# DefTruth/CUDA-Learn-Notes

Hardware: NVIDIA H100
Metric: hgemm_tflops (higher is better)
Workload: dtype f16 (fp32 accumulate)

## Files before the change

### cuda-learn-notes_b200/csrc/hgemm_wgmma.cu

```cuda
#include "abi_common.cuh"
#include "ptx.cuh"

namespace b200k {

namespace gemm {
constexpr int BM = 128, BN = 256, STAGES = 4, THREADS = 384, GROUP_M = 16;
constexpr int STG_BYTES = 16384;
}

template <int DT_, bool A_MN_, bool B_MN_>
struct GemmCfg {
  static constexpr int DT = DT_;
  static constexpr bool A_MN = A_MN_, B_MN = B_MN_;
  static constexpr int ES = DT == 2 ? 4 : 2;
  static constexpr int BK = 128 / ES;
  static constexpr int KSTEP = DT == 2 ? 8 : 16;
  static constexpr int A_BYTES = gemm::BM * BK * ES;
  static constexpr int B_BYTES = gemm::BN * BK * ES;
  static constexpr int STAGE_BYTES = A_BYTES + B_BYTES;
  static constexpr int SMEM_BYTES = gemm::STAGES * STAGE_BYTES + 2 * gemm::STG_BYTES + 1024 + 2 * gemm::STAGES * 8;
  static_assert(!(DT == 2 && (A_MN || B_MN)), "tf32 wgmma reads K-major operands only");
  static_assert(SMEM_BYTES <= 232448, "more shared memory than an H100 block may use");
};

template <class Cfg>
__device__ __forceinline__ void gemm_mma_kblock(float* d, uint32_t sA, uint32_t sB, int cw) {
  constexpr int STEPS = Cfg::BK / Cfg::KSTEP;
#pragma unroll
  for (int k = 0; k < STEPS; ++k) {
    const uint64_t da = Cfg::A_MN ? wgmma_desc(sA + cw * 64 * Cfg::BK * Cfg::ES + k * 2048, 64 * Cfg::BK * Cfg::ES, 1024)
                                  : wgmma_desc(sA + cw * 64 * 128 + k * 32, 16, 1024);
    const uint64_t db = Cfg::B_MN ? wgmma_desc(sB + k * 2048, 64 * Cfg::BK * Cfg::ES, 1024) : wgmma_desc(sB + k * 32, 16, 1024);
    wgmma_ss<Cfg::DT, 256, Cfg::A_MN, Cfg::B_MN>(d, da, db, 1);
  }
}

template <class Cfg>
__device__ __forceinline__ void gemm_store_tile(const float* d, const CUtensorMap* tmC, uint32_t stg, int cw, int row0,
                                                int col0) {
  constexpr int SLICES = Cfg::DT == 2 ? 4 : 2, JS = 32 / SLICES, JB = JS / 2;
  const int t = threadIdx.x & 127, lane = t & 31, warp = t / 32;
  const bool leader = t == 0;
#pragma unroll
  for (int sl = 0; sl < SLICES; ++sl) {
    if (leader) tma_store_wait_read<0>();
    named_bar_sync(1 + cw, 128);
    if constexpr (Cfg::DT == 2) {
      const int q = lane & 3;
#pragma unroll
      for (int jj = 0; jj < JS; ++jj) {
        const int j = sl * JS + jj;
#pragma unroll
        for (int h = 0; h < 2; ++h) {
          const int r = warp * 16 + 8 * h + lane / 4;
          const int chunk = 2 * (jj % JB) + q / 2;
          const uint32_t a = stg + (jj / JB) * 8192 + r * 128 + ((chunk ^ (r & 7)) << 4) + (q & 1) * 8;
          asm volatile("st.shared.v2.f32 [%0], {%1, %2};" ::"r"(a), "f"(d[4 * j + 2 * h]), "f"(d[4 * j + 2 * h + 1])
                       : "memory");
        }
      }
    } else {
      const int m = lane / 8, r = warp * 16 + 8 * (m & 1) + (lane & 7);
#pragma unroll
      for (int jj = 0; jj < JS; jj += 2) {
        const int j = sl * JS + jj, chunk = jj % JB + (m >> 1);
        const uint32_t a = stg + (jj / JB) * 8192 + r * 128 + ((chunk ^ (r & 7)) << 4);
        uint32_t p[4];
#pragma unroll
        for (int i = 0; i < 4; ++i)
          p[i] = Cfg::DT == 1 ? pack_bf162(d[4 * j + 2 * i], d[4 * j + 2 * i + 1])
                              : pack_half2(d[4 * j + 2 * i], d[4 * j + 2 * i + 1]);
        stmatrix_x4(a, p[0], p[1], p[2], p[3]);
      }
    }
    fence_proxy_async_smem();
    named_bar_sync(1 + cw, 128);
    if (leader) {
      const int c = col0 + sl * (gemm::BN / SLICES);
      tma_store_2d(tmC, stg, c, row0);
      tma_store_2d(tmC, stg + 8192, c + 128 / Cfg::ES, row0);
      tma_store_commit();
    }
  }
}

template <class Cfg>
__global__ void __launch_bounds__(gemm::THREADS, 1)
    hgemm_wgmma_kernel(const __grid_constant__ CUtensorMap tmA, const __grid_constant__ CUtensorMap tmB,
                       const __grid_constant__ CUtensorMap tmC, int K, int tiles_m, int tiles_n) {
  using namespace gemm;
  extern __shared__ uint8_t smem_raw[];
  const uint32_t base = (smem_u32(smem_raw) + 1023) & ~1023u;
  const uint32_t stg0 = base + STAGES * Cfg::STAGE_BYTES;
  const uint32_t full0 = stg0 + 2 * STG_BYTES, empty0 = full0 + STAGES * 8;
  const int wg = threadIdx.x / 128;

  const int tile = blockIdx.x, width = GROUP_M * tiles_n, g = tile / width, first_m = g * GROUP_M;
  const int gsz = min(tiles_m - first_m, GROUP_M);
  const int tm = first_m + (tile % width) % gsz, tn = (tile % width) / gsz;
  const int nkb = (K + Cfg::BK - 1) / Cfg::BK;

  if (threadIdx.x == 0) {
    for (int s = 0; s < STAGES; ++s) {
      mbar_init(full0 + 8 * s, 1);
      mbar_init(empty0 + 8 * s, 2);
    }
    fence_mbar_init();
  }
  __syncthreads();

  if (wg == 0) {
    if (threadIdx.x == 0) {
      tma_prefetch_desc(&tmA);
      tma_prefetch_desc(&tmB);
      for (int kb = 0; kb < nkb; ++kb) {
        const int s = kb % STAGES;
        if (kb >= STAGES) mbar_wait_nocall(empty0 + 8 * s, ((kb / STAGES) - 1) & 1);
        const uint32_t bar = full0 + 8 * s, sA = base + s * Cfg::STAGE_BYTES, sB = sA + Cfg::A_BYTES;
        mbar_arrive_expect_tx(bar, Cfg::STAGE_BYTES);
        if constexpr (Cfg::A_MN) {
#pragma unroll
          for (int c = 0; c < BM / 64; ++c)
            tma_load_2d(sA + c * 64 * Cfg::BK * Cfg::ES, &tmA, bar, tm * BM + c * 64, kb * Cfg::BK, kPolicyEvictNormal);
        } else {
          tma_load_2d(sA, &tmA, bar, kb * Cfg::BK, tm * BM, kPolicyEvictNormal);
        }
        if constexpr (Cfg::B_MN) {
#pragma unroll
          for (int c = 0; c < BN / 64; ++c)
            tma_load_2d(sB + c * 64 * Cfg::BK * Cfg::ES, &tmB, bar, tn * BN + c * 64, kb * Cfg::BK, kPolicyEvictNormal);
        } else {
          tma_load_2d(sB, &tmB, bar, kb * Cfg::BK, tn * BN, kPolicyEvictNormal);
        }
      }
    }
    return;
  }

  const int cw = wg - 1, t = threadIdx.x & 127;
  const bool leader = t == 0;
  if (leader) tma_prefetch_desc(&tmC);
  float d[128];
#pragma unroll
  for (int i = 0; i < 128; ++i) d[i] = 0.f;
  for (int kb = 0; kb < nkb; ++kb) {
    const int s = kb % STAGES;
    mbar_wait_nocall(full0 + 8 * s, (kb / STAGES) & 1);
    const uint32_t sA = base + s * Cfg::STAGE_BYTES, sB = sA + Cfg::A_BYTES;
    fence_regs<128>(d);
    wgmma_fence();
    gemm_mma_kblock<Cfg>(d, sA, sB, cw);
    wgmma_commit();
    wgmma_wait<1>();
    fence_regs<128>(d);
    if (kb > 0 && leader) mbar_arrive(empty0 + 8 * ((kb - 1) % STAGES));
  }
  wgmma_wait<0>();
  fence_regs<128>(d);
  gemm_store_tile<Cfg>(d, &tmC, stg0 + cw * STG_BYTES, cw, tm * BM + cw * 64, tn * BN);
  if (leader) tma_store_wait_all<0>();
}

template <class Cfg>
static int launch_gemm(const void* A, const void* B, void* C, int64_t M, int64_t N, int64_t K, cudaStream_t s,
                       const DeviceInfo& di) {
  using namespace gemm;
  auto tmap = [](CUtensorMap* m, const void* p, int64_t rows, int64_t cols, uint32_t box_rows, uint32_t box_cols) {
    const uint64_t dims[2] = {uint64_t(cols), uint64_t(rows)}, strides[1] = {uint64_t(cols) * Cfg::ES};
    const uint32_t box[2] = {box_cols, box_rows};
    return make_tmap(m, p, Cfg::ES, 2, dims, strides, box);
  };
  CUtensorMap tmA, tmB, tmC;
  int rc = Cfg::A_MN ? tmap(&tmA, A, K, M, Cfg::BK, 64) : tmap(&tmA, A, M, K, BM, Cfg::BK);
  if (rc) return rc;
  rc = Cfg::B_MN ? tmap(&tmB, B, K, N, Cfg::BK, 64) : tmap(&tmB, B, N, K, BN, Cfg::BK);
  if (rc) return rc;
  if ((rc = tmap(&tmC, C, M, N, 64, 128 / Cfg::ES))) return rc;
  const int64_t tiles_m = (M + BM - 1) / BM, tiles_n = (N + BN - 1) / BN, tiles = tiles_m * tiles_n;
  if (tiles > INT32_MAX) return set_error(B200K_ESHAPE, "GEMM too large: %lld tiles", (long long)tiles);
  auto kern = hgemm_wgmma_kernel<Cfg>;
  if ((rc = ensure_dynamic_smem(reinterpret_cast<const void*>(kern), di.device, Cfg::SMEM_BYTES))) return rc;
  kern<<<unsigned(tiles), THREADS, Cfg::SMEM_BYTES, s>>>(tmA, tmB, tmC, int(K), int(tiles_m), int(tiles_n));
  B200K_CHECK_CUDA(cudaGetLastError());
  return B200K_OK;
}

template <int DT>
static int gemm_dispatch(const char* who, const void* A, const void* B, void* C, int64_t M, int64_t N, int64_t K,
                         int b_is_nk, int variant, void* stream, int a_is_km = 0) {
  constexpr int PACK = (DT == 2) ? 4 : 8;
  if (!A || !B || !C) return set_error(B200K_EARG, "%s: null pointer", who);
  if (reinterpret_cast<uintptr_t>(C) & 15) return set_error(B200K_EALIGN, "%s: C (%p) must be 16-byte aligned", who, C);
  if (M < 1 || N < 1 || K < 1 || M > INT32_MAX || N > INT32_MAX || K > INT32_MAX)
    return set_error(B200K_ESHAPE, "%s: M,N,K must be in [1, 2^31) (got %lld,%lld,%lld)", who, (long long)M, (long long)N,
                     (long long)K);
  if ((K % PACK) || (N % PACK))
    return set_error(B200K_ESHAPE, "%s: K and N must be multiples of %d (16-byte rows), got K=%lld N=%lld", who, PACK,
                     (long long)K, (long long)N);
  if (a_is_km && DT == 2) return set_error(B200K_EDTYPE, "%s: A stored as [K,M] is built for f16 / bf16 only", who);
  if (a_is_km && (M % PACK))
    return set_error(B200K_ESHAPE, "%s: M must be a multiple of %d when A is stored as [K,M]", who, PACK);
  const int v = variant & 0xff;
  if (v < B200K_HGEMM_AUTO || v > B200K_HGEMM_2CTA_512x256)
    return set_error(B200K_EARG, "%s: variant %d unknown", who, v);
  DeviceInfo di;
  int rc = get_device_info(&di);
  if (rc) return rc;
  cudaStream_t s = static_cast<cudaStream_t>(stream);
  const bool nn = (b_is_nk == 0);
  if constexpr (DT == 2) {
    if (!nn) return launch_gemm<GemmCfg<2, false, false>>(A, B, C, M, N, K, s, di);
    void* bt = nullptr;
    B200K_CHECK_CUDA(cudaMallocAsync(&bt, size_t(K) * size_t(N) * 4, s));
    rc = b200k_mat_transpose_f32(B, bt, K, N, stream);
    if (!rc) rc = launch_gemm<GemmCfg<2, false, false>>(A, bt, C, M, N, K, s, di);
    cudaError_t e = cudaFreeAsync(bt, s);
    if (!rc && e != cudaSuccess) rc = set_error(B200K_ECUDA, "cudaFreeAsync failed: %s", cudaGetErrorString(e));
    return rc;
  } else {
    if (a_is_km)
      return nn ? launch_gemm<GemmCfg<DT, true, true>>(A, B, C, M, N, K, s, di)
                : launch_gemm<GemmCfg<DT, true, false>>(A, B, C, M, N, K, s, di);
    return nn ? launch_gemm<GemmCfg<DT, false, true>>(A, B, C, M, N, K, s, di)
              : launch_gemm<GemmCfg<DT, false, false>>(A, B, C, M, N, K, s, di);
  }
}

}

extern "C" int b200k_hgemm_f16(const void* A, const void* B, void* C, int64_t M, int64_t N, int64_t K, int b_is_nk,
                               int variant, void* stream) {
  return b200k::gemm_dispatch<0>("b200k_hgemm_f16", A, B, C, M, N, K, b_is_nk, variant, stream);
}

extern "C" int b200k_gemm_ex(const void* A, const void* B, void* C, int64_t M, int64_t N, int64_t K, int a_is_km, int b_is_nk,
                             int dtype, int variant, void* stream) {
  switch (dtype) {
    case B200K_F16: return b200k::gemm_dispatch<0>("b200k_gemm_ex(f16)", A, B, C, M, N, K, b_is_nk, variant, stream, a_is_km);
    case B200K_BF16: return b200k::gemm_dispatch<1>("b200k_gemm_ex(bf16)", A, B, C, M, N, K, b_is_nk, variant, stream, a_is_km);
    case B200K_F32: return b200k::gemm_dispatch<2>("b200k_gemm_ex(tf32)", A, B, C, M, N, K, b_is_nk, variant, stream, a_is_km);
    default: return b200k::set_error(B200K_EDTYPE, "b200k_gemm_ex: dtype %d not supported (f16, bf16, f32-as-tf32)", dtype);
  }
}

extern "C" int b200k_gemm(const void* A, const void* B, void* C, int64_t M, int64_t N, int64_t K, int b_is_nk, int dtype,
                          int variant, void* stream) {
  switch (dtype) {
    case B200K_F16: return b200k::gemm_dispatch<0>("b200k_gemm(f16)", A, B, C, M, N, K, b_is_nk, variant, stream);
    case B200K_BF16: return b200k::gemm_dispatch<1>("b200k_gemm(bf16)", A, B, C, M, N, K, b_is_nk, variant, stream);
    case B200K_F32: return b200k::gemm_dispatch<2>("b200k_gemm(tf32)", A, B, C, M, N, K, b_is_nk, variant, stream);
    default: return b200k::set_error(B200K_EDTYPE, "b200k_gemm: dtype %d not supported (f16, bf16, f32-as-tf32)", dtype);
  }
}
```

### cuda-learn-notes_b200/csrc/ptx.cuh

```cuda
#pragma once
#include <cstdint>
#include <cuda.h>
#include <cuda_bf16.h>
#include <cuda_fp16.h>
#include <cuda_runtime.h>

namespace b200k {

#ifndef B200K_SPIN_LIMIT_CYCLES
#define B200K_SPIN_LIMIT_CYCLES (10LL * 1000 * 1000 * 1000)
#endif

__device__ __forceinline__ uint32_t smem_u32(const void* p) {
  return static_cast<uint32_t>(__cvta_generic_to_shared(p));
}
__device__ __forceinline__ void named_bar_sync(uint32_t id, uint32_t nthreads) {
  asm volatile("bar.sync %0, %1;" ::"r"(id), "r"(nthreads) : "memory");
}

__device__ __forceinline__ void mbar_init(uint32_t bar, uint32_t count) {
  asm volatile("mbarrier.init.shared::cta.b64 [%0], %1;" ::"r"(bar), "r"(count) : "memory");
}
__device__ __forceinline__ void fence_mbar_init() {
  asm volatile("fence.mbarrier_init.release.cluster;" ::: "memory");
}
__device__ __forceinline__ void fence_proxy_async_smem() {
  asm volatile("fence.proxy.async.shared::cta;" ::: "memory");
}
__device__ __forceinline__ void mbar_arrive(uint32_t bar) {
  asm volatile("mbarrier.arrive.shared::cta.b64 _, [%0];" ::"r"(bar) : "memory");
}
__device__ __forceinline__ void mbar_arrive_expect_tx(uint32_t bar, uint32_t bytes) {
  asm volatile("mbarrier.arrive.expect_tx.shared::cta.b64 _, [%0], %1;" ::"r"(bar), "r"(bytes) : "memory");
}
__device__ __forceinline__ uint32_t mbar_try_wait(uint32_t bar, uint32_t parity) {
  uint32_t ok;
  asm volatile(
      "{\n\t"
      ".reg .pred P1;\n\t"
      "mbarrier.try_wait.parity.shared::cta.b64 P1, [%1], %2;\n\t"
      "selp.u32 %0, 1, 0, P1;\n\t"
      "}"
      : "=r"(ok)
      : "r"(bar), "r"(parity)
      : "memory");
  return ok;
}
static __device__ __noinline__ void mbar_timeout_trap(uint32_t bar, uint32_t parity) {
  printf("[b200k] mbarrier wait timed out: block (%d,%d) thread %d bar 0x%x parity %u\n", blockIdx.x, blockIdx.y,
         threadIdx.x, bar, parity);
  __trap();
}
__device__ __forceinline__ void mbar_wait(uint32_t bar, uint32_t parity) {
  if (mbar_try_wait(bar, parity)) return;
  long long t0 = clock64();
  while (!mbar_try_wait(bar, parity)) {
    if (clock64() - t0 > B200K_SPIN_LIMIT_CYCLES) mbar_timeout_trap(bar, parity);
  }
}
__device__ __forceinline__ void mbar_wait_nocall(uint32_t bar, uint32_t parity) {
  if (mbar_try_wait(bar, parity)) return;
  long long t0 = clock64();
  while (!mbar_try_wait(bar, parity)) {
    if (clock64() - t0 > B200K_SPIN_LIMIT_CYCLES) asm volatile("trap;");
  }
}

__device__ __forceinline__ void tma_prefetch_desc(const CUtensorMap* m) {
  asm volatile("prefetch.tensormap [%0];" ::"l"(reinterpret_cast<uint64_t>(m)) : "memory");
}
constexpr uint64_t kPolicyEvictNormal = 0x1000000000000000ull;
constexpr uint64_t kPolicyEvictFirst = 0x12F0000000000000ull;

__device__ __forceinline__ void tma_load_2d(uint32_t dst_smem, const CUtensorMap* m, uint32_t bar, int32_t c0,
                                            int32_t c1, uint64_t policy) {
  asm volatile(
      "cp.async.bulk.tensor.2d.shared::cluster.global.mbarrier::complete_tx::bytes.L2::cache_hint"
      " [%0], [%1, {%3, %4}], [%2], %5;" ::"r"(dst_smem),
      "l"(reinterpret_cast<uint64_t>(m)), "r"(bar), "r"(c0), "r"(c1), "l"(policy)
      : "memory");
}
__device__ __forceinline__ void tma_load_3d(uint32_t dst_smem, const CUtensorMap* m, uint32_t bar, int32_t c0,
                                            int32_t c1, int32_t c2, uint64_t policy) {
  asm volatile(
      "cp.async.bulk.tensor.3d.shared::cluster.global.mbarrier::complete_tx::bytes.L2::cache_hint"
      " [%0], [%1, {%3, %4, %5}], [%2], %6;" ::"r"(dst_smem),
      "l"(reinterpret_cast<uint64_t>(m)), "r"(bar), "r"(c0), "r"(c1), "r"(c2), "l"(policy)
      : "memory");
}
__device__ __forceinline__ void tma_store_2d(const CUtensorMap* m, uint32_t src_smem, int32_t c0, int32_t c1) {
  asm volatile("cp.async.bulk.tensor.2d.global.shared::cta.bulk_group [%0, {%2, %3}], [%1];" ::"l"(
                   reinterpret_cast<uint64_t>(m)),
               "r"(src_smem), "r"(c0), "r"(c1)
               : "memory");
}
__device__ __forceinline__ void tma_store_commit() { asm volatile("cp.async.bulk.commit_group;" ::: "memory"); }
template <int N>
__device__ __forceinline__ void tma_store_wait_read() {
  asm volatile("cp.async.bulk.wait_group.read %0;" ::"n"(N) : "memory");
}
template <int N>
__device__ __forceinline__ void tma_store_wait_all() {
  asm volatile("cp.async.bulk.wait_group %0;" ::"n"(N) : "memory");
}
__device__ __forceinline__ void stmatrix_x4(uint32_t addr, uint32_t r0, uint32_t r1, uint32_t r2, uint32_t r3) {
  asm volatile("stmatrix.sync.aligned.m8n8.x4.shared.b16 [%0], {%1, %2, %3, %4};" ::"r"(addr), "r"(r0), "r"(r1), "r"(r2),
               "r"(r3)
               : "memory");
}

__device__ __forceinline__ uint64_t wgmma_desc(uint32_t smem_addr, uint32_t lbo, uint32_t sbo) {
  return uint64_t((smem_addr & 0x3FFFF) >> 4) | (uint64_t(lbo >> 4) << 16) | (uint64_t(sbo >> 4) << 32) | (1ull << 62);
}
__device__ __forceinline__ void wgmma_fence() { asm volatile("wgmma.fence.sync.aligned;" ::: "memory"); }
__device__ __forceinline__ void wgmma_commit() { asm volatile("wgmma.commit_group.sync.aligned;" ::: "memory"); }
template <int N>
__device__ __forceinline__ void wgmma_wait() { asm volatile("wgmma.wait_group.sync.aligned %0;" ::"n"(N) : "memory"); }
template <int N>
__device__ __forceinline__ void fence_regs(float* d) {
#pragma unroll
  for (int i = 0; i < N; ++i) asm volatile("" : "+f"(d[i])::"memory");
}

#define B200K_ACC8(i) \
  "+f"(d[i]), "+f"(d[i + 1]), "+f"(d[i + 2]), "+f"(d[i + 3]), "+f"(d[i + 4]), "+f"(d[i + 5]), "+f"(d[i + 6]), "+f"(d[i + 7])
#define B200K_ACC32(i) B200K_ACC8(i), B200K_ACC8(i + 8), B200K_ACC8(i + 16), B200K_ACC8(i + 24)
#define B200K_ACC64 B200K_ACC32(0)
#define B200K_ACC128 B200K_ACC64, B200K_ACC32(32)
#define B200K_ACC192 B200K_ACC128, B200K_ACC32(64)
#define B200K_ACC256 B200K_ACC192, B200K_ACC32(96)
#define B200K_PH64 \
  "%0, %1, %2, %3, %4, %5, %6, %7, %8, %9, %10, %11, %12, %13, %14, %15, " \
  "%16, %17, %18, %19, %20, %21, %22, %23, %24, %25, %26, %27, %28, %29, %30, %31"
#define B200K_PH128 \
  B200K_PH64 ", %32, %33, %34, %35, %36, %37, %38, %39, %40, %41, %42, %43, %44, %45, %46, %47, " \
  "%48, %49, %50, %51, %52, %53, %54, %55, %56, %57, %58, %59, %60, %61, %62, %63"
#define B200K_PH192 \
  B200K_PH128 ", %64, %65, %66, %67, %68, %69, %70, %71, %72, %73, %74, %75, %76, %77, %78, %79, " \
  "%80, %81, %82, %83, %84, %85, %86, %87, %88, %89, %90, %91, %92, %93, %94, %95"
#define B200K_PH256 \
  B200K_PH192 ", %96, %97, %98, %99, %100, %101, %102, %103, %104, %105, %106, %107, %108, %109, %110, %111, " \
  "%112, %113, %114, %115, %116, %117, %118, %119, %120, %121, %122, %123, %124, %125, %126, %127"
#define B200K_WGMMA(shape, type, acc, scale, ops) \
  "{\n.reg .pred p;\nsetp.ne.b32 p, " scale ", 0;\n" \
  "wgmma.mma_async.sync.aligned." shape ".f32." type " {" acc "}, " ops ";\n}\n"
#define B200K_SS(type, n, scale, ops) \
  asm volatile(B200K_WGMMA("m64n" #n "k16", type, B200K_PH##n, scale, ops) \
               : B200K_ACC##n \
               : "l"(da), "l"(db), "r"(scale_d), "n"(TA), "n"(TB))
#define B200K_RS(type, n, scale, ops) \
  asm volatile(B200K_WGMMA("m64n" #n "k16", type, B200K_PH##n, scale, ops) \
               : B200K_ACC##n \
               : "r"(a[0]), "r"(a[1]), "r"(a[2]), "r"(a[3]), "l"(db), "r"(scale_d), "n"(TB))
#define B200K_F16_OR_BF16(op, ...) \
  if constexpr (DT == 0) \
    op("f16.f16", __VA_ARGS__); \
  else \
    op("bf16.bf16", __VA_ARGS__)

template <int DT, int N, int TA, int TB>
__device__ __forceinline__ void wgmma_ss(float* d, uint64_t da, uint64_t db, int scale_d) {
  static_assert(N == 64 || N == 128 || N == 256, "wgmma_ss: N must be 64, 128 or 256");
  static_assert(DT == 0 || DT == 1 || (DT == 2 && N == 256 && TA == 0 && TB == 0),
                "wgmma_ss: f16 / bf16, or tf32 with N = 256 and K-major operands");
  if constexpr (DT == 2) {
    asm volatile(B200K_WGMMA("m64n256k8", "tf32.tf32", B200K_PH256, "%130", "%128, %129, p, 1, 1")
                 : B200K_ACC256
                 : "l"(da), "l"(db), "r"(scale_d));
  } else if constexpr (N == 64) {
    B200K_F16_OR_BF16(B200K_SS, 64, "%34", "%32, %33, p, 1, 1, %35, %36");
  } else if constexpr (N == 128) {
    B200K_F16_OR_BF16(B200K_SS, 128, "%66", "%64, %65, p, 1, 1, %67, %68");
  } else {
    B200K_F16_OR_BF16(B200K_SS, 256, "%130", "%128, %129, p, 1, 1, %131, %132");
  }
}
template <int DT, int N, int TB>
__device__ __forceinline__ void wgmma_rs(float* d, const uint32_t* a, uint64_t db, int scale_d) {
  static_assert(N == 64 || N == 128 || N == 192 || N == 256, "wgmma_rs: N must be 64, 128, 192 or 256");
  static_assert(DT == 0 || DT == 1, "wgmma_rs: f16 or bf16");
  if constexpr (N == 64) {
    B200K_F16_OR_BF16(B200K_RS, 64, "%37", "{%32, %33, %34, %35}, %36, p, 1, 1, %38");
  } else if constexpr (N == 128) {
    B200K_F16_OR_BF16(B200K_RS, 128, "%69", "{%64, %65, %66, %67}, %68, p, 1, 1, %70");
  } else if constexpr (N == 192) {
    B200K_F16_OR_BF16(B200K_RS, 192, "%101", "{%96, %97, %98, %99}, %100, p, 1, 1, %102");
  } else {
    B200K_F16_OR_BF16(B200K_RS, 256, "%133", "{%128, %129, %130, %131}, %132, p, 1, 1, %134");
  }
}
#undef B200K_ACC8
#undef B200K_ACC32
#undef B200K_ACC64
#undef B200K_ACC128
#undef B200K_ACC192
#undef B200K_ACC256
#undef B200K_PH64
#undef B200K_PH128
#undef B200K_PH192
#undef B200K_PH256
#undef B200K_WGMMA
#undef B200K_SS
#undef B200K_RS
#undef B200K_F16_OR_BF16

__device__ __forceinline__ uint32_t pack_half2(float lo, float hi) {
  __half2 h = __floats2half2_rn(lo, hi);
  return *reinterpret_cast<uint32_t*>(&h);
}
__device__ __forceinline__ uint32_t pack_bf162(float lo, float hi) {
  __nv_bfloat162 h = __floats2bfloat162_rn(lo, hi);
  return *reinterpret_cast<uint32_t*>(&h);
}

}
```

Measured before the change: 758.5.

## Pair CTAs in 2-wide clusters and multicast shared B tiles via TMA

Launches the GEMM with 2-CTA clusters along M when the M tile count is even. The two CTAs share the same N tile, so each loads half of the B tile and multicasts it into both CTAs' shared memory. Stage release becomes cluster-wide: consumers arrive on their own empty barrier and on the peer's. The producer waits at the end so shared memory is not freed while the peer is still writing. This is meant to halve the L2 and global read traffic for B. The cost is cross-CTA synchronisation, cluster scheduling limits, and the two CTAs stalling each other.

```diff
diff --git a/cuda-learn-notes_b200/csrc/hgemm_wgmma.cu b/cuda-learn-notes_b200/csrc/hgemm_wgmma.cu
--- a/cuda-learn-notes_b200/csrc/hgemm_wgmma.cu
+++ b/cuda-learn-notes_b200/csrc/hgemm_wgmma.cu
@@ -99,15 +99,17 @@
   const int gsz = min(tiles_m - first_m, GROUP_M);
   const int tm = first_m + (tile % width) % gsz, tn = (tile % width) / gsz;
   const int nkb = (K + Cfg::BK - 1) / Cfg::BK;
+  const uint32_t rank = cluster_ctarank(), ncta = cluster_nctarank();
+  const bool pair = ncta == 2;
 
   if (threadIdx.x == 0) {
     for (int s = 0; s < STAGES; ++s) {
       mbar_init(full0 + 8 * s, 1);
-      mbar_init(empty0 + 8 * s, 2);
+      mbar_init(empty0 + 8 * s, 2 * ncta);
     }
     fence_mbar_init();
   }
-  __syncthreads();
+  cluster_sync_after_mbar_init();
 
   if (wg == 0) {
     if (threadIdx.x == 0) {
@@ -127,12 +129,24 @@
         }
         if constexpr (Cfg::B_MN) {
 #pragma unroll
-          for (int c = 0; c < BN / 64; ++c)
-            tma_load_2d(sB + c * 64 * Cfg::BK * Cfg::ES, &tmB, bar, tn * BN + c * 64, kb * Cfg::BK, kPolicyEvictNormal);
+          for (int c = 0; c < BN / 64; ++c) {
+            const uint32_t dst = sB + c * 64 * Cfg::BK * Cfg::ES;
+            if (!pair)
+              tma_load_2d(dst, &tmB, bar, tn * BN + c * 64, kb * Cfg::BK, kPolicyEvictNormal);
+            else if (c / (BN / 128) == int(rank))
+              tma_load_2d_multicast(dst, &tmB, bar, tn * BN + c * 64, kb * Cfg::BK, 0x3, kPolicyEvictNormal);
+          }
         } else {
-          tma_load_2d(sB, &tmB, bar, kb * Cfg::BK, tn * BN, kPolicyEvictNormal);
+          if (!pair) {
+            tma_load_2d(sB, &tmB, bar, kb * Cfg::BK, tn * BN, kPolicyEvictNormal);
+          } else {
+            const int row = rank * (BN / 2);
+            tma_load_2d_multicast(sB + row * Cfg::BK * Cfg::ES, &tmB, bar, kb * Cfg::BK, tn * BN + row, 0x3,
+                                  kPolicyEvictNormal);
+          }
         }
       }
+      for (int s = 0; s < min(nkb, STAGES); ++s) mbar_wait_nocall(empty0 + 8 * s, ((nkb - 1 - s) / STAGES) & 1);
     }
     return;
   }
@@ -140,6 +154,11 @@
   const int cw = wg - 1, t = threadIdx.x & 127;
   const bool leader = t == 0;
   if (leader) tma_prefetch_desc(&tmC);
+  auto release = [&](int s) {
+    if (!leader) return;
+    mbar_arrive(empty0 + 8 * s);
+    if (pair) mbar_arrive_cluster(mapa(empty0 + 8 * s, rank ^ 1));
+  };
   float d[128];
 #pragma unroll
   for (int i = 0; i < 128; ++i) d[i] = 0.f;
@@ -153,10 +172,11 @@
     wgmma_commit();
     wgmma_wait<1>();
     fence_regs<128>(d);
-    if (kb > 0 && leader) mbar_arrive(empty0 + 8 * ((kb - 1) % STAGES));
+    if (kb > 0) release((kb - 1) % STAGES);
   }
   wgmma_wait<0>();
   fence_regs<128>(d);
+  release((nkb - 1) % STAGES);
   gemm_store_tile<Cfg>(d, &tmC, stg0 + cw * STG_BYTES, cw, tm * BM + cw * 64, tn * BN);
   if (leader) tma_store_wait_all<0>();
 }
@@ -170,18 +190,29 @@
     const uint32_t box[2] = {box_cols, box_rows};
     return make_tmap(m, p, Cfg::ES, 2, dims, strides, box);
   };
+  const int64_t tiles_m = (M + BM - 1) / BM, tiles_n = (N + BN - 1) / BN, tiles = tiles_m * tiles_n;
+  if (tiles > INT32_MAX) return set_error(B200K_ESHAPE, "GEMM too large: %lld tiles", (long long)tiles);
+  const unsigned ncta = tiles_m % 2 == 0 ? 2 : 1;
   CUtensorMap tmA, tmB, tmC;
   int rc = Cfg::A_MN ? tmap(&tmA, A, K, M, Cfg::BK, 64) : tmap(&tmA, A, M, K, BM, Cfg::BK);
   if (rc) return rc;
-  rc = Cfg::B_MN ? tmap(&tmB, B, K, N, Cfg::BK, 64) : tmap(&tmB, B, N, K, BN, Cfg::BK);
+  rc = Cfg::B_MN ? tmap(&tmB, B, K, N, Cfg::BK, 64) : tmap(&tmB, B, N, K, BN / ncta, Cfg::BK);
   if (rc) return rc;
   if ((rc = tmap(&tmC, C, M, N, 64, 128 / Cfg::ES))) return rc;
-  const int64_t tiles_m = (M + BM - 1) / BM, tiles_n = (N + BN - 1) / BN, tiles = tiles_m * tiles_n;
-  if (tiles > INT32_MAX) return set_error(B200K_ESHAPE, "GEMM too large: %lld tiles", (long long)tiles);
   auto kern = hgemm_wgmma_kernel<Cfg>;
   if ((rc = ensure_dynamic_smem(reinterpret_cast<const void*>(kern), di.device, Cfg::SMEM_BYTES))) return rc;
-  kern<<<unsigned(tiles), THREADS, Cfg::SMEM_BYTES, s>>>(tmA, tmB, tmC, int(K), int(tiles_m), int(tiles_n));
-  B200K_CHECK_CUDA(cudaGetLastError());
+  cudaLaunchAttribute cluster;
+  cluster.id = cudaLaunchAttributeClusterDimension;
+  cluster.val.clusterDim.x = ncta;
+  cluster.val.clusterDim.y = cluster.val.clusterDim.z = 1;
+  cudaLaunchConfig_t cfg = {};
+  cfg.gridDim = dim3(unsigned(tiles));
+  cfg.blockDim = dim3(THREADS);
+  cfg.dynamicSmemBytes = Cfg::SMEM_BYTES;
+  cfg.stream = s;
+  cfg.attrs = &cluster;
+  cfg.numAttrs = 1;
+  B200K_CHECK_CUDA(cudaLaunchKernelEx(&cfg, kern, tmA, tmB, tmC, int(K), int(tiles_m), int(tiles_n)));
   return B200K_OK;
 }
 
diff --git a/cuda-learn-notes_b200/csrc/ptx.cuh b/cuda-learn-notes_b200/csrc/ptx.cuh
--- a/cuda-learn-notes_b200/csrc/ptx.cuh
+++ b/cuda-learn-notes_b200/csrc/ptx.cuh
@@ -18,6 +18,25 @@
   asm volatile("bar.sync %0, %1;" ::"r"(id), "r"(nthreads) : "memory");
 }
 
+__device__ __forceinline__ uint32_t cluster_ctarank() {
+  uint32_t r;
+  asm volatile("mov.u32 %0, %%cluster_ctarank;" : "=r"(r));
+  return r;
+}
+__device__ __forceinline__ uint32_t cluster_nctarank() {
+  uint32_t n;
+  asm volatile("mov.u32 %0, %%cluster_nctarank;" : "=r"(n));
+  return n;
+}
+__device__ __forceinline__ uint32_t mapa(uint32_t local_smem_addr, uint32_t rank) {
+  uint32_t r;
+  asm volatile("mapa.shared::cluster.u32 %0, %1, %2;" : "=r"(r) : "r"(local_smem_addr), "r"(rank));
+  return r;
+}
+__device__ __forceinline__ void cluster_sync_after_mbar_init() {
+  asm volatile("barrier.cluster.arrive.relaxed.aligned;\n\tbarrier.cluster.wait.acquire.aligned;" ::: "memory");
+}
+
 __device__ __forceinline__ void mbar_init(uint32_t bar, uint32_t count) {
   asm volatile("mbarrier.init.shared::cta.b64 [%0], %1;" ::"r"(bar), "r"(count) : "memory");
 }
@@ -29,6 +48,9 @@
 }
 __device__ __forceinline__ void mbar_arrive(uint32_t bar) {
   asm volatile("mbarrier.arrive.shared::cta.b64 _, [%0];" ::"r"(bar) : "memory");
+}
+__device__ __forceinline__ void mbar_arrive_cluster(uint32_t cluster_bar) {
+  asm volatile("mbarrier.arrive.shared::cluster.b64 _, [%0];" ::"r"(cluster_bar) : "memory");
 }
 __device__ __forceinline__ void mbar_arrive_expect_tx(uint32_t bar, uint32_t bytes) {
   asm volatile("mbarrier.arrive.expect_tx.shared::cta.b64 _, [%0], %1;" ::"r"(bar), "r"(bytes) : "memory");
@@ -78,6 +100,14 @@
       "cp.async.bulk.tensor.2d.shared::cluster.global.mbarrier::complete_tx::bytes.L2::cache_hint"
       " [%0], [%1, {%3, %4}], [%2], %5;" ::"r"(dst_smem),
       "l"(reinterpret_cast<uint64_t>(m)), "r"(bar), "r"(c0), "r"(c1), "l"(policy)
+      : "memory");
+}
+__device__ __forceinline__ void tma_load_2d_multicast(uint32_t dst_smem, const CUtensorMap* m, uint32_t bar, int32_t c0,
+                                                      int32_t c1, uint16_t cta_mask, uint64_t policy) {
+  asm volatile(
+      "cp.async.bulk.tensor.2d.shared::cluster.global.mbarrier::complete_tx::bytes.multicast::cluster.L2::cache_hint"
+      " [%0], [%1, {%3, %4}], [%2], %5, %6;" ::"r"(dst_smem),
+      "l"(reinterpret_cast<uint64_t>(m)), "r"(bar), "r"(c0), "r"(c1), "h"(cta_mask), "l"(policy)
       : "memory");
 }
 __device__ __forceinline__ void tma_load_3d(uint32_t dst_smem, const CUtensorMap* m, uint32_t bar, int32_t c0,
```

Result: no change. 756.4 (median of 6 runs) (-0.3%).
